# TeemoCaption/FDDM-asr

Hardware: AMD Instinct MI355X
Metric: train-step utterances/sec (10 s @16 kHz, seq_len 256) at 1/2/4/8 MI355X (higher is better)
Workload: dtype bf16; 1 GPU; fddm_zhTW_base C2: WavLM-base + 6L d512 H8 ff2048 decoder, V=8000, T=200, dropout 0.1, n_step_fd=4; global_batch=32, seq_len=256, parallelism=dp1

## Files before the change

fddm-asr_amd/csrc/attention.hip:

```cpp
#include "attn_common.h"

namespace fddm {
namespace attn {


template <typename T> struct Cfg;
template <> struct Cfg<bf16_t> { static constexpr int RB = 128, NSUB = 2, ECH = 8; };
template <> struct Cfg<float> { static constexpr int RB = 256, NSUB = 4, ECH = 4; };

__device__ __forceinline__ int hatt(int k) { return ((k >> 1) & 3) << 2; }

template <typename T>
__device__ __forceinline__ void mma(f32x4_t& c, const uint4& a, const uint4& b);
template <> __device__ __forceinline__ void mma<bf16_t>(f32x4_t& c, const uint4& a, const uint4& b) {
  c = __builtin_amdgcn_mfma_f32_16x16x32_bf16(__builtin_bit_cast(bf16x8_t, a), __builtin_bit_cast(bf16x8_t, b), c, 0, 0, 0);
}
template <> __device__ __forceinline__ void mma<float>(f32x4_t& c, const uint4& a, const uint4& b) {
  c = __builtin_amdgcn_mfma_f32_16x16x4f32(__uint_as_float(a.x), __uint_as_float(b.x), c, 0, 0, 0);
  c = __builtin_amdgcn_mfma_f32_16x16x4f32(__uint_as_float(a.y), __uint_as_float(b.y), c, 0, 0, 0);
  c = __builtin_amdgcn_mfma_f32_16x16x4f32(__uint_as_float(a.z), __uint_as_float(b.z), c, 0, 0, 0);
  c = __builtin_amdgcn_mfma_f32_16x16x4f32(__uint_as_float(a.w), __uint_as_float(b.w), c, 0, 0, 0);
}

template <typename T>
// ... 2197 lines not shown
        uv.y = pk(kok ? dv[d][2] * vsc : 0.f, kok ? dv[d][3] * vsc : 0.f);
        *(uint2*)(dKb + d * 16 + 4 * g) = uk;
        *(uint2*)(dVb + d * 16 + 4 * g) = uv;
      }
    }
  }
  ASTAMP(12);
#ifdef ATTN_STAMPS
  asm volatile("s_waitcnt vmcnt(0)" ::: "memory");
#endif
  ASTAMP(13);
  ARTIME(15);
}

static int g_attn_v6 = 0;
#ifndef A7_FUSED_MAXLQ
#define A7_FUSED_MAXLQ 256
#endif
static bool attn7_enabled() { return g_attn_v6 != 1; }

static int g_last_fwd = AF_NONE, g_last_bwd = AB_NONE;
void attn_note_fwd(int kernel, int dm, int mk, bool kx, bool rel) {
  g_last_fwd = kernel | (dm << 4) | (mk << 6) | ((int)kx << 8) | ((int)rel << 9);
}
void attn_note_bwd(int kernel, int dm, int mk, int np, bool kx) {
  g_last_bwd = kernel | (dm << 4) | (mk << 6) | (np << 9) | ((int)kx << 11);
}
void attn_note_dkv(int kernel, int dm, bool mask, bool kx) {
  const bool same = ((g_last_bwd >> 4) & 3) == dm && (((g_last_bwd >> 11) & 1) != 0) == kx;
  g_last_bwd |= ((same ? kernel : (int)AB_DISAGREE) << 12) | ((int)mask << 8);
// ... 7 lines not shown
      n = v;
    else
      n = 256;
  }
  return n;
}

template <typename T>
static int run(int which, AttnArgs& a, hipStream_t s) {
  constexpr int RB = Cfg<T>::RB;
  const bool drop = a.thr16 != 0, mask = a.key_keep != nullptr || (a.Lk % 64) != 0;
  if constexpr (sizeof(T) == 2) {
    if (which == 0) {
      const bool rel = a.table != nullptr && (a.gate != nullptr || a.graw != nullptr || a.gx != nullptr);
      const int LkP = (a.Lk + 63) / 64 * 64;
      if (rel) {
        if (drop) return (int)hipErrorInvalidValue;
        if (attn7_enabled() && a.Lk <= 1024 && g_attn_v6 != 5) return attn7_fwd(a, s);
        const size_t lds5 = (size_t)2 * 2 * 64 * 128 + (size_t)LkP * 4 + (size_t)(LkP + 128) * 4;
        dim3 grid5((a.Lq + 127) / 128, a.B * a.H);
        if (mask) hipLaunchKernelGGL((fwd5_kernel<true, 2, 2>), grid5, dim3(256), lds5, s, a);
        else hipLaunchKernelGGL((fwd5_kernel<false, 2, 2>), grid5, dim3(256), lds5, s, a);
        attn_note_fwd(AF_FWD5, 0, mask, false, true);
        return (int)hipGetLastError();
      }
      if (a.Lk <= 1024) {
        const int ntiles = LkP / 64, qw = 128;
        const int dm = !drop ? 0 : (a.bits_ready && a.dbits) ? 1 : 2;
        if (attn7_enabled() && (dm != 2 || a.dbits)) {
          if (dm == 2) {
            const int e = attn7_drop_bits(a.dbits, 0, 1, a.B * a.H, a.Lq, a.Lk, a.seed, a.stream, 0, a.thr16,
                                          a.seed_off, s);
            if (e) return e;
// ... 133 lines not shown
FDDM_API int fddm_attn_stamps(unsigned long long* host, long n) {
  return (int)hipMemcpyFromSymbol(host, HIP_SYMBOL(fddm::attn::attn_stamps), n * sizeof(unsigned long long), 0,
                                  hipMemcpyDeviceToHost);
}
FDDM_API int fddm_attn_stamps_clear() {
  static unsigned long long z[8192 * 16];
  return (int)hipMemcpyToSymbol(HIP_SYMBOL(fddm::attn::attn_stamps), z, sizeof(z), 0, hipMemcpyHostToDevice);
}
#endif

FDDM_API int fddm_attn_last_path(void) { return (int)((unsigned)g_last_fwd | ((unsigned)g_last_bwd << 16)); }

FDDM_API int fddm_attn_set_kernels(int v6) {
  const int old = g_attn_v6;
  g_attn_v6 = (v6 >= 1 && v6 <= 5) ? v6 : 0;
  return old;
}

static int attn_fwd_impl(int dtype, const void* Q, long sq, const void* K, long sk, const void* V, long sv, void* O,
                         long so, float* lse, const unsigned char* key_keep, const int* key_len, const float* gate,
                         const float* table, int B, int H, int Lq, int Lk, float scale, float drop_p,
                         unsigned long long seed, unsigned long long stream, unsigned long long* drop_bits,
                         int drop_bits_ready, void* hs) {
  if (table && !gate) return (int)hipErrorInvalidValue;
  attn_note_fwd(AF_NONE, 0, 0, false, false);
  AttnArgs a{};
  a.key_len = key_len;
  a.dbits = (uint64_t*)drop_bits;
  a.bits_ready = drop_bits_ready;
  a.Q = Q; a.K = K; a.V = V; a.Out = O; a.lse = lse;
// ... 130 lines not shown
```

fddm-asr_amd/csrc/attn8.hip:

```cpp
#include "attn7_common.h"

namespace fddm {
namespace attn {

constexpr int A8_NS = 4;
#ifndef A8_RSMFMA
#define A8_RSMFMA 1
#endif
#ifndef A8_WPS
#define A8_WPS 2
#endif

__device__ __forceinline__ void pinv(float& x) { asm volatile("" : "+v"(x)); }
__device__ __forceinline__ void pinv(unsigned& x) { asm volatile("" : "+v"(x)); }
template <int B0, int B1>
__device__ __forceinline__ unsigned keep_pack(float x, float y, unsigned kw) {
  unsigned r, t;
  asm volatile(
      "v_bfe_i32 %1, %3, %5, 1\n\t"
      "v_and_b32 %1, %1, %2\n\t"
      "v_bfe_i32 %0, %3, %6, 1\n\t"
      "v_and_b32 %0, %0, %4\n\t"
      "v_cvt_pk_bf16_f32 %0, %1, %0"
      : "=&v"(r), "=&v"(t)
      : "v"(x), "v"(kw), "v"(y), "i"(B0), "i"(B1));
  return r;
}
#define A8_FENCE() __builtin_amdgcn_sched_barrier(0)

#ifdef A8_STAMPS
#define A8ST(k)                                 \
  do {                                          \
    a8st_[k] = __builtin_amdgcn_s_memtime();  \
  } while (0)
#else
#define A8ST(k) \
  do {          \
  } while (0)
#endif
#if defined(A8_STAMPS) && defined(A8_FINE)
#define A8FS(k)                                                  \
  do {                                                           \
    if (a8pc_ == A8_FINE) a8fs_[k] = __builtin_amdgcn_s_memtime(); \
  } while (0)
#else
#define A8FS(k) \
  do {          \
  } while (0)
#endif

__host__ __device__ __forceinline__ int attn8_fwd_fb_off(int Lk) {
  const int LkP = (Lk + 63) / 64 * 64;
  return (2 * A8_NS * A7_TB + A8_NS * 512 * 4 + 16 + LkP * 4 + 15) / 16 * 16;
}

template <int DM, int MK>
__global__ void __launch_bounds__(256, A8_WPS) fwd8_kernel(AttnArgs a) {
  constexpr bool DROP = DM != 0;
  constexpr int NP = DROP ? 6 : 4;
  extern __shared__ __attribute__((aligned(16))) unsigned char sm8[];
  const int ntiles = (a.Lk + 63) >> 6, LkP = ntiles * 64;
  unsigned char* kst = sm8;
  unsigned char* vst = sm8 + A8_NS * A7_TB;
  unsigned* kbl = (unsigned*)(sm8 + 2 * A8_NS * A7_TB);
  unsigned* mpk = kbl + A8_NS * 512 + 4;
  const int tid = threadIdx.x, lane = tid & 63, w = __builtin_amdgcn_readfirstlane(tid >> 6);
  const int hh = lane >> 5, qi = lane & 31;
  int bxi, bh;
  xcd_tile(bxi, bh);
#ifdef A8_STAMPS
  unsigned long long a8st_[16] = {};
#endif
#if defined(A8_STAMPS) && defined(A8_FINE)
  unsigned long long a8fs_[16] = {};
  int a8pc_ = 0;
#endif
  A8ST(0);
  const int b = bh / a.H, h = bh - b * a.H;
  const int qw0 = bxi * 256 + 64 * w;
  const bf16_t* Qb = (const bf16_t*)a.Q + (long)b * a.Lq * a.sq + h * DH;
  const bf16_t* Kb = (const bf16_t*)a.K + (long)b * a.Lk * a.sk + h * DH;
  const bf16_t* Vb = (const bf16_t*)a.V + (long)b * a.Lk * a.sv + h * DH;
  const unsigned sk2 = (unsigned)a.sk * 2u, sv2 = (unsigned)a.sv * 2u;
  const int nqg = (a.Lq + 31) >> 5, qg0 = 8 * bxi + 2 * w;
  const unsigned* lbits = (const unsigned*)(a.dbits + (long)a.B * a.H * nqg * ntiles * 32);

  unsigned kb8[4] = {1u, 1u, 1u, 1u};
  if constexpr (MK == 2) {
#pragma unroll
    for (int j = 0; j < 4; ++j) {
      const int k = min(4 * tid + j, a.Lk - 1);
      asm volatile("global_load_ubyte %0, %1, off" : "=v"(kb8[j]) : "v"(a.key_keep + (long)b * a.Lk + k) : "memory");
    }
  }
  const int qA = qw0 + qi, qB = qw0 + 32 + qi;
  unsigned char* qst = sm8 + attn8_fwd_fb_off(a.Lk) + w * 16384;
#pragma unroll
  for (int u = 0; u < 8; ++u) {
    const int r = 8 * u + (lane >> 3), pch = lane & 7;
    const unsigned qr = (unsigned)min(qw0 + r, a.Lq - 1);
    dma16_sv(Qb, qr * (unsigned)a.sq * 2u + (unsigned)((pch ^ (r & 7)) << 4), qst + 8 * u * 128);
  }
  const unsigned tmask = ntiles >= 32 ? 0xFFFFFFFFu : ((1u << ntiles) - 1u);
  const int nact = ntiles;
  A8ST(15);

  const unsigned kst_a = lds_addr(kst), vst_a = lds_addr(vst), kbl_a = lds_addr(kbl);
  auto piece = [&](int tt, int st, int k) {
    if (k < 4) {
      const int u = k >> 1, R = 16 * w + 8 * u;
      const int r0 = R + (lane >> 3), pch = lane & 7;
// ... 5 lines not shown
    } else {
      const int c = k - 4;
      dma4_so(lbits, (unsigned)(lb_dword(bh, nqg, ntiles, min(qg0 + c, nqg - 1), tt) + lane) * 4u,
              kbl_a + (st * 512 + (2 * w + c) * 64) * 4);
    }
  };
  unsigned fmask = tmask;
  int flast = 0;
  auto next_fill_tile = [&]() {
    if (fmask) {
      flast = __builtin_ctz(fmask);
      fmask &= fmask - 1u;
    }
    return flast;
  };
  {
    const int t0 = next_fill_tile(), t1 = next_fill_tile();
#pragma unroll
    for (int k = 0; k < NP; ++k) piece(t0, 0, k);
#pragma unroll
    for (int k = 0; k < NP; ++k) piece(t1, 1, k);
  }
  A8ST(11);
  asm volatile("s_waitcnt vmcnt(%4)" : "+v"(kb8[0]), "+v"(kb8[1]), "+v"(kb8[2]), "+v"(kb8[3]) : "n"(NP) : "memory");
  if constexpr (MK != 0) {
    if (4 * tid < LkP) {
      unsigned mv[4];
#pragma unroll
      for (int j = 0; j < 4; ++j) {
        const bool ok = 4 * tid + j < a.Lk && (MK == 1 || (kb8[j] & 0xFFu) != 0);
        mv[j] = pk_bf16(1.f, ok ? 0.f : -INFINITY);
      }
      *(uint4*)(mpk + 4 * tid) = make_uint4(mv[0], mv[1], mv[2], mv[3]);
    }
  }
  __builtin_amdgcn_s_barrier();
  A8ST(1);
  const float sl2 = a.scale * 1.4426950408889634f;
  uint4 qa[4], qb[4];
  {
    const unsigned zA = qA < a.Lq ? 0xFFFFFFFFu : 0u, zB = qB < a.Lq ? 0xFFFFFFFFu : 0u;
    const int rA = qi, rB = qi + 32;
#pragma unroll
    for (int ks = 0; ks < 4; ++ks) {
      const uint4 x = *(const uint4*)(qst + rA * 128 + (((2 * ks + hh) ^ (rA & 7)) << 4));
      const uint4 y = *(const uint4*)(qst + rB * 128 + (((2 * ks + hh) ^ (rB & 7)) << 4));
      qa[ks] = scale_frag(make_uint4(x.x & zA, x.y & zA, x.z & zA, x.w & zA), sl2);
      qb[ks] = scale_frag(make_uint4(y.x & zB, y.y & zB, y.z & zB, y.w & zB), sl2);
    }
  }

  int koff[4];
#pragma unroll
  for (int ks = 0; ks < 4; ++ks) koff[ks] = qi * 128 + (((2 * ks + hh) ^ ((qi >> 1) & 7)) << 4);
  const int vi = lane & 15, vrow = 4 * hh + (vi >> 2);
  int voff[2];
#pragma unroll
  for (int db = 0; db < 2; ++db)
    voff[db] = vrow * 128 + (((8 * db + 4 * ((lane >> 4) & 1) + (vi & 3)) ^ ((vrow & 2) << 2)) << 3);

  float rfA = 0.f, rfB = 0.f;
  f32x16_t oA0 = {}, oA1 = {}, oB0 = {}, oB1 = {};
  constexpr bool RSM = A8_RSMFMA != 0;
  float lsA = 0.f, lsB = 0.f;
  f32x16_t lsum = {};
  uint4 ucar = make_uint4(0, 0, 0, 0);
  const unsigned one2 = 0x3F803F80u, selA1 = qi < 16 ? one2 : 0u, selB1 = qi < 16 ? 0u : one2;
  const uint4 selA = make_uint4(selA1, selA1, selA1, selA1), selB = make_uint4(selB1, selB1, selB1, selB1);
  f32x16_t sA, sB;
  uint4 pA[2], pB[2];
  pB[0] = pB[1] = make_uint4(0, 0, 0, 0);
  const uint4 q5init = hh ? make_uint4(0, 0, 0, 0) : make_uint4(pk_bf16(0.f, 1.f), 0u, 0u, 0u);
  uint4 q5A = q5init, q5B = q5init;
  unsigned kwA = 0xFFFFFFFFu, kwB = 0xFFFFFFFFu;
  uint4 kf[4], vf[2][2];
  uint4 k5 = make_uint4(0, 0, 0, 0);
  const unsigned lo32 = hh ? 0u : 0xFFFFFFFFu;
  auto mk5 = [&](int key0) {
    unsigned mk = pk_bf16(1.f, 0.f);
    if constexpr (MK != 0) mk = mpk[key0 + qi];
    return make_uint4(mk & lo32, 0u, 0u, 0u);
  };
  unsigned mkr = 0;
  auto mk5_read = [&](int key0) {
    if constexpr (MK != 0) mkr = mpk[key0 + qi];
  };
  auto mk5_set = [&]() {
    unsigned mk = pk_bf16(1.f, 0.f);
    if constexpr (MK != 0) mk = mkr;
    k5 = make_uint4(mk & lo32, 0u, 0u, 0u);
// ... 28 lines not shown
    if constexpr (DROP) v = keep_pack<lb_bit(kb, 2 * i), lb_bit(kb, 2 * i + 1)>(x, y, kw);
    else v = pk_bf16(x, y);
    pset(p, ic, v);
  };
  auto first_ref = [&](const f32x16_t& s, float& rf, uint4& q5) {
    float tm = fmaxf(s[0], s[1]);
#pragma unroll
    for (int r = 2; r < 16; r += 2) tm = fmaxf(tm, fmaxf(s[r], s[r + 1]));
    tm = xmax32(tm);
    rf = (tm == -INFINITY) ? 0.f : __uint_as_float(((unsigned)pk_bf16(tm, 0.f)) << 16);
    q5 = hh ? make_uint4(0, 0, 0, 0) : make_uint4(pk_bf16(-rf, 1.f), 0u, 0u, 0u);
  };

  auto phase = [&](f32x16_t& SX, const uint4 (&qX)[4], const uint4& q5X, f32x16_t& oY0, f32x16_t& oY1,
                   const uint4 (&pY)[2], const f32x16_t& sZ, float dZ, uint4 (&pZ)[2], float& lZ,
                   const uint4& selZ, const uint4& selP, unsigned kwZ, auto kbc, auto&& rd, auto&& dm) {
    constexpr int KB = decltype(kbc)::value;
    float ex[8], ey[8], la, lb;
    unsigned sh[8], u[8], mk[8];
    auto expo = [&](auto ic) {
      constexpr int i = decltype(ic)::value;
#ifndef A8_NOEXP
      ex[i] = __builtin_amdgcn_exp2f(sZ[2 * i] - dZ);
      ey[i] = __builtin_amdgcn_exp2f(sZ[2 * i + 1] - dZ);
#else
      ex[i] = sZ[2 * i] - dZ;
      ey[i] = sZ[2 * i + 1] - dZ;
#endif
      pinv(ex[i]);
      pinv(ey[i]);
      if constexpr (DROP) {
        sh[i] = kwZ << (8 * KB + i);
        pinv(sh[i]);
      }
    };
    auto fin = [&](auto ic) {
      constexpr int i = decltype(ic)::value;
      if constexpr (!RSM) {
        if constexpr (i == 0) {
          la = ex[0];
          lb = ey[0];
        } else {
// ... 14 lines not shown
        pinv(mk[i]);
      } else {
        pset(pZ, ic, u[i]);
      }
    };
    auto apply = [&](auto ic) {
      constexpr int i = decltype(ic)::value;
      if constexpr (DROP) {
        unsigned v = u[i] & mk[i];
        pinv(v);
        pset(pZ, ic, v);
      }
    };
    auto stages = [&](auto cc) {
      constexpr int c = decltype(cc)::value;
      if constexpr (c < 8) expo(std::integral_constant<int, c>{});
      if constexpr (c >= 1) fin(std::integral_constant<int, c - 1>{});
      if constexpr (c >= 2) apply(std::integral_constant<int, c - 2>{});
      if constexpr (c == 8) {
        apply(std::integral_constant<int, 7>{});
        if constexpr (!RSM) lZ += la + lb;
      }
    };
    auto rsum = [&](auto cc) {
      constexpr int c = decltype(cc)::value;
      if constexpr (RSM && c == 1) lsum = mfma32(selP, ucar, lsum);
      if constexpr (RSM && c == 6) lsum = mfma32(selZ, make_uint4(u[0], u[1], u[2], u[3]), lsum);
    };
#if defined(A8_STAMPS) && defined(A8_FINE)
    ++a8pc_;
// ... 16 lines not shown
      A8FS(ks + 2);
    });
    SX = acc;
    static_for<0, 4>([&](auto pc) {
      constexpr int pi = decltype(pc)::value;
      if constexpr ((pi & 1) == 0) oY0 = mfma32(vf[pi >> 1][0], pY[pi >> 1], oY0);
      else oY1 = mfma32(vf[pi >> 1][1], pY[pi >> 1], oY1);
      rsum(std::integral_constant<int, 5 + pi>{});
      stages(std::integral_constant<int, 5 + pi>{});
      rd(std::integral_constant<int, 5 + pi>{});
      dm(std::integral_constant<int, 5 + pi>{});
      A8_FENCE();
      A8FS(pi + 6);
    });
    if constexpr (RSM) ucar = make_uint4(u[4], u[5], u[6], u[7]);
  };

  unsigned cmask = tmask;
  int t = __builtin_ctz(cmask);
  cmask &= cmask - 1u;
  int st = 0;
  if (nact > 0) {
  {
#pragma unroll
    for (int ks = 0; ks < 4; ++ks) kf[ks] = *(const uint4*)(kst + koff[ks]);
    k5 = mk5(64 * t);
    if constexpr (DROP) {
      kwA = kbl[(2 * w) * 64 + lane];
      kwB = kbl[(2 * w + 1) * 64 + lane];
    }
    f32x16_t acc = mfma32(k5, q5A, f32x16_t{});
#pragma unroll
    for (int ks = 0; ks < 4; ++ks) acc = mfma32(kf[ks], qa[ks], acc);
    sA = acc;
#pragma unroll
    for (int c = 0; c < 4; ++c) rdv(vst, c);
  }
  int fidx = 2, ftile = next_fill_tile();
  auto dm_first = [&](auto base, auto cc) {
    constexpr int c = decltype(cc)::value, k = decltype(base)::value + c / 3;
    if constexpr (c % 3 == 1 && k < NP) piece(ftile, fidx & 3, k);
  };
  auto dm_none = [&](auto) {};
  first_ref(sA, rfA, q5A);
  phase(sB, qb, q5B, oB0, oB1, pB, sA, rfA, pA, lsA, selA, selB, kwA, std::integral_constant<int, 0>{},
        [&](auto cc) {
          constexpr int c = decltype(cc)::value;
          if constexpr (c == 1) mk5_read(64 * t + 32);
          if constexpr (c == 8) mk5_set();
          if constexpr (c >= 5) kf[c - 5] = *(const uint4*)(kst + koff[c - 5] + 32 * 128);
        },
        [&](auto cc) { dm_first(std::integral_constant<int, 0>{}, cc); });
  first_ref(sB, rfB, q5B);
  phase(sA, qa, q5A, oA0, oA1, pA, sB, rfB, pB, lsB, selB, selA, kwB, std::integral_constant<int, 0>{},
        [&](auto cc) {
          constexpr int c = decltype(cc)::value;
          if constexpr (c < 4) rdv(vst, c);
        },
        [&](auto cc) { dm_first(std::integral_constant<int, 3>{}, cc); });
  A8ST(2);
  auto dm_span = [&](auto base, auto cc) {
    constexpr int c = decltype(cc)::value, k = decltype(base)::value + (c == 6 ? 1 : 0);
    if constexpr ((c == 2 || c == 6) && k < NP) piece(ftile, fidx & 3, k);
  };
  for (int i = 0;; ++i) {
    const bool more = cmask != 0u;
    int tn = t, stn = st;
    unsigned kwAn = 0xFFFFFFFFu, kwBn = 0xFFFFFFFFu;
    if (more) {
      tn = __builtin_ctz(cmask);
      cmask &= cmask - 1u;
      stn = st == A8_NS - 1 ? 0 : st + 1;
#ifndef A8_NOWAIT
      asm volatile("s_waitcnt vmcnt(%0) lgkmcnt(0)" ::"n"(NP) : "memory");
// ... 16 lines not shown
        kwBn = kbl[stn * 512 + (2 * w + 1) * 64 + lane];
      }
    }
    ++fidx;
    ftile = next_fill_tile();
    {
      const unsigned char* kimn = kst + stn * A7_TB;
      const unsigned char* vimg = vst + st * A7_TB;
      phase(sB, qb, q5B, oB0, oB1, pB, sA, 0.f, pA, lsA, selA, selB, kwA, std::integral_constant<int, 1>{},
            [&](auto cc) {
              constexpr int c = decltype(cc)::value;
              if constexpr (c == 1) mk5_read(64 * tn);
              if constexpr (c == 8) mk5_set();
              if constexpr (c >= 5) kf[c - 5] = *(const uint4*)(kimn + koff[c - 5]);
            },
            [&](auto cc) { dm_span(std::integral_constant<int, 0>{}, cc); });
      phase(sA, qa, q5A, oA0, oA1, pA, sB, 0.f, pB, lsB, selB, selA, kwB, std::integral_constant<int, 1>{},
            [&](auto cc) {
              constexpr int c = decltype(cc)::value;
              if constexpr (c < 4) rdv(vimg + 32 * 128, c);
            },
            [&](auto cc) { dm_span(std::integral_constant<int, 2>{}, cc); });
    }
    if (!more) break;
    t = tn;
    st = stn;
    kwA = kwAn;
    kwB = kwBn;
    {
      const unsigned char* kimg = kst + st * A7_TB;
      const unsigned char* vimg = vst + st * A7_TB;
      phase(sB, qb, q5B, oB0, oB1, pB, sA, 0.f, pA, lsA, selA, selB, kwA, std::integral_constant<int, 0>{},
            [&](auto cc) {
              constexpr int c = decltype(cc)::value;
              if constexpr (c == 1) mk5_read(64 * t + 32);
              if constexpr (c == 8) mk5_set();
              if constexpr (c >= 5) kf[c - 5] = *(const uint4*)(kimg + koff[c - 5] + 32 * 128);
            },
            [&](auto cc) { dm_span(std::integral_constant<int, 4>{}, cc); });
      phase(sA, qa, q5A, oA0, oA1, pA, sB, 0.f, pB, lsB, selB, selA, kwB, std::integral_constant<int, 0>{},
            [&](auto cc) {
              constexpr int c = decltype(cc)::value;
              if constexpr (c < 4) rdv(vimg, c);
            },
            dm_none);
    }
  }
#pragma unroll
  for (int s = 0; s < 2; ++s) {
    oB0 = mfma32(vf[s][0], pB[s], oB0);
    oB1 = mfma32(vf[s][1], pB[s], oB1);
  }
  if constexpr (RSM) lsum = mfma32(selB, ucar, lsum);
  }

  A8ST(12);
  asm volatile("s_waitcnt vmcnt(0)" ::: "memory");
  A8ST(13);
  float ltA = RSM ? lsum[0] : xsum32(lsA), ltB = RSM ? lsum[8] : xsum32(lsB);
#ifdef A8_NOFALLBACK
  if (false) {
#else
  if (nact > 0 && __any(!(ltA <= 0x1p64f && ltA >= 0x1p-40f) || !(ltB <= 0x1p64f && ltB >= 0x1p-40f))) {
#endif
    unsigned char* kp = sm8 + attn8_fwd_fb_off(a.Lk) + w * 16384;
    unsigned char* vp = kp + 8192;
    auto redo = [&](int c, const uint4 (&qX)[4], f32x16_t& o0, f32x16_t& o1, float& l, float& rf) {
      const int qg = min(qg0 + c, nqg - 1);
      float m = -INFINITY;
      rf = 0.f;
      l = 0.f;
      o0 = f32x16_t{};
      o1 = f32x16_t{};
      uint4 q5 = q5init;
      unsigned tm_ = tmask;
      while (tm_) {
        const int tt = __builtin_ctz(tm_);
        tm_ &= tm_ - 1u;
        const int r = 64 * tt + lane, rr = min(r, a.Lk - 1);
#pragma unroll
        for (int ch = 0; ch < 8; ++ch) {
          const uint4 kx = *(const uint4*)(Kb + (long)rr * a.sk + 8 * ch);
          const uint4 vx = *(const uint4*)(Vb + (long)rr * a.sv + 8 * ch);
          *(uint4*)(kp + lane * 128 + ((ch ^ ((lane >> 1) & 7)) << 4)) = kx;
          *(uint4*)(vp + lane * 128 + ((ch ^ vsw(lane)) << 4)) = vx;
        }
        unsigned kw = 0xFFFFFFFFu;
        if constexpr (DROP) kw = lbits[lb_dword(bh, nqg, ntiles, qg, tt) + lane];
        static_for<0, 2>([&](auto kbc) {
          constexpr int kb = decltype(kbc)::value;
          const uint4 k5_ = mk5(64 * tt + 32 * kb);
          f32x16_t sc = mfma32(k5_, q5, f32x16_t{});
#pragma unroll
          for (int ks = 0; ks < 4; ++ks) sc = mfma32(*(const uint4*)(kp + koff[ks] + kb * 32 * 128), qX[ks], sc);
          float tmx = fmaxf(sc[0], sc[1]);
#pragma unroll
          for (int rr2 = 2; rr2 < 16; rr2 += 2) tmx = fmaxf(tmx, fmaxf(sc[rr2], sc[rr2 + 1]));
          tmx = xmax32(tmx) + rf;
          const float mn = fmaxf(m, tmx);
          float rn = rf;
          if (mn != -INFINITY) rn = __uint_as_float(((unsigned)pk_bf16(mn, 0.f)) << 16);
          const float alpha = (m == -INFINITY) ? 0.f : __builtin_amdgcn_exp2f(rf - rn);
          l *= alpha;
          o0 *= alpha;
          o1 *= alpha;
          uint4 pp[2];
          float la = 0.f, lb = 0.f;
          static_for<0, 8>([&](auto ic) { sm_pair_f32(sc, rn - rf, kw, pp, la, lb, kbc, ic); });
          l += la + lb;
          m = mn;
          rf = rn;
          q5 = hh ? make_uint4(0, 0, 0, 0) : make_uint4(pk_bf16(-rf, 1.f), 0u, 0u, 0u);
#pragma unroll
          for (int s = 0; s < 2; ++s) {
            const int rb = (32 * kb + 16 * s) * 128;
            o0 = mfma32(join_tr(tr_read(vp + voff[0] + rb), tr_read(vp + voff[0] + rb + 1024)), pp[s], o0);
            o1 = mfma32(join_tr(tr_read(vp + voff[1] + rb), tr_read(vp + voff[1] + rb + 1024)), pp[s], o1);
          }
        });
      }
      l = xsum32(l);
    };
    redo(0, qa, oA0, oA1, ltA, rfA);
    redo(1, qb, oB0, oB1, ltB, rfB);
  }
  bf16_t* Ob = (bf16_t*)a.Out + (long)b * a.Lq * a.so + h * DH;
#pragma unroll
  for (int c = 0; c < 2; ++c) {
    const float lt = c ? ltB : ltA;
    const float rf = c ? rfB : rfA;
    const float inv = (lt > 0.f) ? (DROP ? a.drop_scale : 1.f) / lt : NAN;
    const int q = qw0 + 32 * c + qi;
    bf16_t* orow = Ob + (long)min(q, a.Lq - 1) * a.so;
#pragma unroll
    for (int db = 0; db < 2; ++db) {
      const f32x16_t& oo = c ? (db ? oB1 : oB0) : (db ? oA1 : oA0);
#pragma unroll
      for (int gp = 0; gp < 2; ++gp) {
        unsigned p0[2], p1[2];
#pragma unroll
        for (int j = 0; j < 2; ++j) {
          p0[j] = pk_bf16(oo[8 * gp + 2 * j] * inv, oo[8 * gp + 2 * j + 1] * inv);
          p1[j] = pk_bf16(oo[8 * gp + 4 + 2 * j] * inv, oo[8 * gp + 4 + 2 * j + 1] * inv);
        }
        const auto s0 = __builtin_amdgcn_permlane32_swap(p0[0], p1[0], false, false);
        const auto s1 = __builtin_amdgcn_permlane32_swap(p0[1], p1[1], false, false);
        const uint4 v = make_uint4(s0[0], s1[0], s0[1], s1[1]);
// ... 10 lines not shown
    unsigned long long* dst = (unsigned long long*)(Ob + (long)(bxi * 256) * a.so);
#pragma unroll
    for (int k = 0; k < 16; ++k) dst[k] = a8st_[k];
#ifdef A8_FINE
    unsigned long long* dst2 = (unsigned long long*)(Ob + (long)(bxi * 256 + 1) * a.so);
#pragma unroll
    for (int k = 0; k < 16; ++k) dst2[k] = a8fs_[k];
#endif
  }
#endif
}

#ifndef A8_LDS_FLOOR
#define A8_LDS_FLOOR 0
#endif
size_t attn8_fwd_lds(int Lk) {
  const size_t n = (size_t)attn8_fwd_fb_off(Lk) + 4 * 16384;
  return n > (size_t)A8_LDS_FLOOR ? n : (size_t)A8_LDS_FLOOR;
}

int attn8_fwd(AttnArgs& a, hipStream_t s) {
  if (a.Lk > 1024 || a.Lk <= 0 || a.Lq <= 0) return (int)hipErrorInvalidValue;
  const int dm = a.thr16 == 0 ? 0 : 1;
  const int mk = a.key_keep != nullptr ? 2 : (a.Lk % 64) != 0 ? 1 : 0;
  const size_t lds = attn8_fwd_lds(a.Lk);
  dim3 grid((a.Lq + 255) / 256, a.B * a.H);
#define FWD8(D, M) hipLaunchKernelGGL((fwd8_kernel<D, M>), grid, dim3(256), lds, s, a)
  if (dm) { if (mk == 2) FWD8(1, 2); else if (mk == 1) FWD8(1, 1); else FWD8(1, 0); }
  else { if (mk == 2) FWD8(0, 2); else if (mk == 1) FWD8(0, 1); else FWD8(0, 0); }
#undef FWD8
  attn_note_fwd(AF_FWD8, dm, mk, false, false);
  return (int)hipGetLastError();
}

}
}
```

fddm-asr_amd/csrc/attn_common.h:

```cpp
#pragma once
#include "common.h"

FDDM_API long fddm_attn_drop_words(int B, int H, int Lq, int Lk);

namespace fddm {
namespace attn {

__device__ __forceinline__ void xcd_tile(int& bx, int& by) {
  const int nx = gridDim.x, n = nx * gridDim.y;
  const int L = blockIdx.x + blockIdx.y * nx;
  const int x = L & 7, j = L >> 3, q = n >> 3, r = n & 7;
  const int W = (x < r ? x * (q + 1) : r * (q + 1) + (x - r) * q) + j;
  by = W / nx;
  bx = W - by * nx;
}


constexpr int DH = 64;

__device__ __forceinline__ int kc_off(int RB, int r, int c) { return r * RB + ((c ^ ((r >> 1) & 7)) << 4); }

__device__ __forceinline__ float xmax16(float x) {
  const auto r = __builtin_amdgcn_permlane16_swap(__float_as_uint(x), __float_as_uint(x), false, false);
  return fmaxf(__uint_as_float(r[0]), __uint_as_float(r[1]));
// ... 59 lines not shown
  asm volatile("s_mov_b32 m0, %1\n\tglobal_load_lds_dwordx4 %0, off" ::"v"(src), "s"(la) : "memory", "m0");
}
__device__ __forceinline__ void pin16(uint4& x) {
  u32x4v_t v = __builtin_bit_cast(u32x4v_t, x);
  asm volatile("" : "+v"(v));
  x = __builtin_bit_cast(uint4, v);
}

enum { AF_NONE = 0, AF_FWD7, AF_FWD8, AF_FWD6, AF_FWD2, AF_FWD5, AF_GENERIC };
enum { AB_NONE = 0, AB_BWDF7, AB_V7, AB_V2, AB_BWD3S, AB_V4, AB_GENERIC, AB_DISAGREE = 15 };
void attn_note_fwd(int kernel, int dm, int mk, bool kx, bool rel);
void attn_note_bwd(int kernel, int dm, int mk, int np, bool kx);
void attn_note_dkv(int kernel, int dm, bool mask, bool kx);

int attn7_fwd(AttnArgs& a, hipStream_t s);
int attn8_fwd(AttnArgs& a, hipStream_t s);
int attn7_dq(AttnArgs& a, hipStream_t s);
int attn7_dkv(AttnArgs& a, hipStream_t s);
int attn7_bwdf(AttnArgs& a, hipStream_t s);
int attn7_drop_bits(uint64_t* out, long site_words, int nsites, int BH, int Lq, int Lk, uint64_t seed,
                    uint64_t stream0, uint64_t stream_step, unsigned thr16, const uint64_t* seed_off, hipStream_t s);
long attn7_drop_words(int B, int H, int Lq, int Lk);

}
}
```

fddm-asr_amd/fddm_hip/_lib.py:

```python
from __future__ import annotations

import ctypes
import os
import re

_HERE = os.path.dirname(os.path.abspath(__file__))
LIB_PATH = os.environ.get("FDDM_HIP_LIB", os.path.join(_HERE, "libfddm_hip.so"))
_HEADER_CANDIDATES = [
    os.path.join(os.path.dirname(os.path.dirname(_HERE)), "include", "fddm_hip.h"),
    os.path.join(os.path.dirname(_HERE), "include", "fddm_hip.h"),
]


def header_path() -> str:
    for p in _HEADER_CANDIDATES:
        if os.path.exists(p):
            return p
    raise FileNotFoundError("include/fddm_hip.h not found next to the package")


def _ctype(t: str):
    t = t.strip()
    if "*" in t:
        return ctypes.c_void_p
# ... 39 lines not shown
    global _lib, _decls
    if _lib is None:
        if not os.path.exists(LIB_PATH):
            raise ImportError(f"libfddm_hip.so not built ({LIB_PATH}); run `make -C fddm-asr_amd` or "
                              "__graft_entry__.build(). There is no CPU fallback.")
        L = ctypes.CDLL(LIB_PATH)
        _decls = parse_header()
        for name, (res, args) in _decls.items():
            f = getattr(L, name)
            f.restype = res
            f.argtypes = args
        _lib = L
        ak = os.environ.get("FDDM_ATTN_KERNELS")
        if ak:
            L.fddm_attn_set_kernels({"auto": 0, "v6": 1, "nofused": 2, "fwd7": 3, "fwd8": 4, "relfwd5": 5}[ak])
    return _lib


def declared_symbols():
    return sorted(parse_header().keys())


def call(name: str, *args):
    f = getattr(lib(), name)
    rc = f(*args)
    if rc != 0:
        msg = lib().fddm_error_string(rc)
        raise RuntimeError(f"{name} failed: hipError {rc} ({msg.decode() if msg else '?'})")
    return rc
```

include/fddm_hip.h:

```cpp
#ifndef FDDM_HIP_H
#define FDDM_HIP_H
#ifdef __cplusplus
extern "C" {
#endif

int fddm_abi_version(void);
const char* fddm_error_string(int code);

int fddm_gemm(int dtype, int a_dtype, int a_kc, int b_kc, int epi, int out_dtype, const void* A, long lda, long Mi,
              long sAb, const void* B, long ldb, void* C, long ldc, void* C2, const float* bias, float alpha, long M,
              long N, long K, unsigned long long seed, unsigned long long stream, float drop_p, float* colsum,
              void* hip_stream);

int fddm_linear_dx_rope(const void* dy, long ldy, const void* w, long ldw, float* dx, long lddx, const float* cs,
                        const float* sn, long M, long N, long K, long L, void* hip_stream);

int fddm_gemm_persistent_cap(int cap);

int fddm_gemm_dw_grouped(int n, const void* const* dy, const long* ldy, const void* const* x, const long* ldx,
                         float* const* dw, const long* lddw, float* const* db, const long* M, const long* N,
                         const long* K, long kchunk, void* hip_stream);

int fddm_conv1d_gemm(int dtype, int epi, const void* x, long lda, long sAb, long Tin, long Cg, long cstride,
                     long cpad, const void* W, void* out, long ldc, const float* bias, long Bn, long Tout, long N,
// ... 97 lines not shown
                     void* hip_stream);
int fddm_lfd_std_bwd(int zt_dtype, const float* dzt, const void* zt, const float* inv_std, float* dz, long B, long C,
                     void* hip_stream);
int fddm_lfd_loss(const float* Cm, float* loss, long D, float lam, void* hip_stream);
int fddm_lfd_dloss(int out_dtype, const float* Cm, const float* gscale, void* dC, long D, float lam, void* hip_stream);
int fddm_lfd_colstat(const float* z, float* out, const float* mean_sum, float inv_n, long B, long C, void* hip_stream);
int fddm_lfd_std_apply(int out_dtype, const float* z, void* zt, float* inv_std, const float* s1, const float* s2,
                       float inv_n, float eps, long B, long C, void* hip_stream);
int fddm_lfd_bwd_colstat(int zt_dtype, const float* dzt, const void* zt, float* out, long B, long C, void* hip_stream);
int fddm_lfd_std_bwd_apply(int zt_dtype, const float* dzt, const void* zt, const float* inv_std, const float* sums,
                           float inv_n, float scale, float* dz, long B, long C, void* hip_stream);

int fddm_gemm_force_path(int path);
int fddm_gemm_last_path(void);
int fddm_attn_set_kernels(int v6);
int fddm_attn_last_path(void);


int fddm_set_seed_offset(const unsigned long long* off);

int fddm_grad_sumsq(const long* chunk_tensor, const long* chunk_start, const long* numel, const float* const* g,
                    long nchunks, float* total, void* hip_stream);
int fddm_adamw(const long* chunk_tensor, const long* chunk_start, const long* numel, float* const* p,
               const float* const* g, float* const* m, float* const* v, unsigned short* const* pbf,
               float* const* step, long ntensors, long nchunks, const float* total, float max_norm, float lr,
               float lr_wd, float b1, float b2, float eps, int* skipped, int zero_g, float grad_scale,
               void* hip_stream);

int fddm_rows_mean(int dtype, const void* x, float* out, long B, long S, long d, void* hip_stream);
int fddm_time_embed(const long* t, float* emb, long B, long d, float max_steps, void* hip_stream);
// ... 22 lines not shown
```

Before: 3425 utterances/s.

## Add relative-position-bias variant of fwd8 attention kernel for WavLM gated bias

```diff
diff --git a/fddm-asr_amd/csrc/attention.hip b/fddm-asr_amd/csrc/attention.hip
--- a/fddm-asr_amd/csrc/attention.hip
+++ b/fddm-asr_amd/csrc/attention.hip
@@ -2235,6 +2235,7 @@
 }
 
 static int g_attn_v6 = 0;
+static int g_wavlm_fwd = 0;
 #ifndef A7_FUSED_MAXLQ
 #define A7_FUSED_MAXLQ 256
 #endif
@@ -2272,9 +2273,18 @@
     if (which == 0) {
       const bool rel = a.table != nullptr && (a.gate != nullptr || a.graw != nullptr || a.gx != nullptr);
       const int LkP = (a.Lk + 63) / 64 * 64;
+      if (a.table != nullptr && !rel) return (int)hipErrorInvalidValue;
       if (rel) {
         if (drop) return (int)hipErrorInvalidValue;
-        if (attn7_enabled() && a.Lk <= 1024 && g_attn_v6 != 5) return attn7_fwd(a, s);
+        if (attn7_enabled() && a.Lk <= 1024 && g_attn_v6 != 5) {
+          const bool can8 = !a.key_keep && !a.key_len && a.gx && !a.gate && !a.graw && a.Lk <= A8_REL_MAXLK &&
+                            a.Lq <= a.Lk;
+          const long nh = (long)a.B * a.H, ncu = attn_cu_count();
+          const long load8 = (nh * ((a.Lq + 255) / 256) + ncu - 1) / ncu * 256;
+          const long load7 = (nh * ((a.Lq + 127) / 128) + ncu - 1) / ncu * 128;
+          const bool use8 = can8 && g_attn_v6 != 3 && g_wavlm_fwd == 0 && (g_attn_v6 == 4 || load8 <= load7);
+          return use8 ? attn8_fwd(a, s) : attn7_fwd(a, s);
+        }
         const size_t lds5 = (size_t)2 * 2 * 64 * 128 + (size_t)LkP * 4 + (size_t)(LkP + 128) * 4;
         dim3 grid5((a.Lq + 127) / 128, a.B * a.H);
         if (mask) hipLaunchKernelGGL((fwd5_kernel<true, 2, 2>), grid5, dim3(256), lds5, s, a);
@@ -2438,6 +2448,12 @@
 FDDM_API int fddm_attn_set_kernels(int v6) {
   const int old = g_attn_v6;
   g_attn_v6 = (v6 >= 1 && v6 <= 5) ? v6 : 0;
+  return old;
+}
+
+FDDM_API int fddm_attn_set_wavlm_fwd(int fwd7_only) {
+  const int old = g_wavlm_fwd;
+  g_wavlm_fwd = fwd7_only == 1 ? 1 : 0;
   return old;
 }
 
diff --git a/fddm-asr_amd/csrc/attn8.hip b/fddm-asr_amd/csrc/attn8.hip
--- a/fddm-asr_amd/csrc/attn8.hip
+++ b/fddm-asr_amd/csrc/attn8.hip
@@ -28,6 +28,24 @@
 }
 #define A8_FENCE() __builtin_amdgcn_sched_barrier(0)
 
+__device__ __forceinline__ u32x4v_t gload16(const void* p) {
+  u32x4v_t v;
+  asm volatile("global_load_dwordx4 %0, %1, off" : "=v"(v) : "v"(p) : "memory");
+  return v;
+}
+__device__ __forceinline__ unsigned gload4(const void* p) {
+  unsigned v;
+  asm volatile("global_load_dword %0, %1, off" : "=v"(v) : "v"(p) : "memory");
+  return v;
+}
+__device__ __forceinline__ void pin4v(u32x4v_t& x) { asm volatile("" : "+v"(x)); }
+typedef unsigned a8_u32x2 __attribute__((ext_vector_type(2)));
+__device__ __forceinline__ a8_u32x2 lds_ld64(unsigned a) {
+  typedef __attribute__((address_space(3))) const volatile a8_u32x2* lp_t;
+  return *(lp_t)(size_t)a;
+}
+constexpr int A8_BPAD = 288;
+
 #ifdef A8_STAMPS
 #define A8ST(k)                                 \
   do {                                          \
@@ -54,8 +72,9 @@
   return (2 * A8_NS * A7_TB + A8_NS * 512 * 4 + 16 + LkP * 4 + 15) / 16 * 16;
 }
 
-template <int DM, int MK>
+template <int DM, int MK, bool REL = false>
 __global__ void __launch_bounds__(256, A8_WPS) fwd8_kernel(AttnArgs a) {
+  static_assert(!REL || (DM == 0 && MK != 2), "the bias build has no dropout and no key-padding bytes");
   constexpr bool DROP = DM != 0;
   constexpr int NP = DROP ? 6 : 4;
   extern __shared__ __attribute__((aligned(16))) unsigned char sm8[];
@@ -63,7 +82,7 @@
   unsigned char* kst = sm8;
   unsigned char* vst = sm8 + A8_NS * A7_TB;
   unsigned* kbl = (unsigned*)(sm8 + 2 * A8_NS * A7_TB);
-  unsigned* mpk = kbl + A8_NS * 512 + 4;
+  unsigned* mpk = kbl + (REL ? 0 : A8_NS * 512) + 4;
   const int tid = threadIdx.x, lane = tid & 63, w = __builtin_amdgcn_readfirstlane(tid >> 6);
   const int hh = lane >> 5, qi = lane & 31;
   int bxi, bh;
@@ -94,7 +113,7 @@
     }
   }
   const int qA = qw0 + qi, qB = qw0 + 32 + qi;
-  unsigned char* qst = sm8 + attn8_fwd_fb_off(a.Lk) + w * 16384;
+  unsigned char* qst = REL ? (w < 2 ? kst : vst) + (2 + (w & 1)) * A7_TB : sm8 + attn8_fwd_fb_off(a.Lk) + w * 16384;
 #pragma unroll
   for (int u = 0; u < 8; ++u) {
     const int r = 8 * u + (lane >> 3), pch = lane & 7;
@@ -130,10 +149,35 @@
     }
     return flast;
   };
+  constexpr int CLP = REL ? A8_BPAD : 0;
+  const int CL = LkP + CLP;
+  float* bcp = (float*)(mpk + LkP);
+  u32x4v_t gxr[2][4], gwr[2][8];
+  auto rel_loads = [&]() {
+    if constexpr (REL) {
+#pragma unroll
+      for (int c = 0; c < 2; ++c) {
+        const long qc = min(qw0 + 32 * c + qi, a.Lq - 1);
+        const bf16_t* xr = (const bf16_t*)a.gx + ((long)b * a.Lq + qc) * a.sgx + h * DH + 32 * hh;
+#pragma unroll
+        for (int u = 0; u < 4; ++u) gxr[c][u] = gload16(xr + 8 * u);
+#pragma unroll
+        for (int u = 0; u < 8; ++u) gwr[c][u] = gload16(a.gw + 64 * c + 32 * hh + 4 * u);
+      }
+      const float* tabh = a.table + (long)h * (2 * a.Lk - 1);
+      const unsigned bcp_a = lds_addr(bcp);
+      for (int g = w; g < 2 * CL / 64; g += 4) {
+        const int i = 64 * g + lane, c = i >= CL ? 1 : 0;
+        const int ti = (a.Lk - 1) - (bxi * 256 + 255) + (i - c * CL) + c;
+        dma4_so(tabh, (unsigned)min(max(ti, 0), 2 * a.Lk - 2) * 4u, bcp_a + 256u * (unsigned)g);
+      }
+    }
+  };
   {
     const int t0 = next_fill_tile(), t1 = next_fill_tile();
 #pragma unroll
     for (int k = 0; k < NP; ++k) piece(t0, 0, k);
+    rel_loads();
 #pragma unroll
     for (int k = 0; k < NP; ++k) piece(t1, 1, k);
   }
@@ -150,8 +194,48 @@
       *(uint4*)(mpk + 4 * tid) = make_uint4(mv[0], mv[1], mv[2], mv[3]);
     }
   }
+  float g2A = 0.f, g2B = 0.f;
+  unsigned blA = 0, blB = 0;
+  auto bias_off = [&](int c) {
+    const int jq = 255 - (64 * w + 32 * c + qi);
+    return (jq & 1) * CL + (jq & ~1) + 4 * hh;
+  };
   __builtin_amdgcn_s_barrier();
   A8ST(1);
+  if constexpr (REL) {
+#pragma unroll
+    for (int c = 0; c < 2; ++c) {
+#pragma unroll
+      for (int u = 0; u < 4; ++u) pin4v(gxr[c][u]);
+#pragma unroll
+      for (int u = 0; u < 8; ++u) pin4v(gwr[c][u]);
+    }
+    const float ba = a.gw[128], bb = a.gw[129], gc = a.gconst[h];
+    auto gate2 = [&](const u32x4v_t (&xv)[4], bool qv) {
+      float sa = 0.f, sb = 0.f;
+#pragma unroll
+      for (int c = 0; c < 4; ++c) {
+#pragma unroll
+        for (int j = 0; j < 2; ++j) {
+          const u32x4v_t A = gwr[0][2 * c + j], Bw = gwr[1][2 * c + j];
+          const float e0 = __uint_as_float(xv[c][2 * j] << 16), e1 = __uint_as_float(xv[c][2 * j] & 0xFFFF0000u);
+          const float e2 = __uint_as_float(xv[c][2 * j + 1] << 16), e3 = __uint_as_float(xv[c][2 * j + 1] & 0xFFFF0000u);
+          sa = fmaf(e0, __uint_as_float(A[0]), fmaf(e1, __uint_as_float(A[1]), fmaf(e2, __uint_as_float(A[2]),
+                                                                                    fmaf(e3, __uint_as_float(A[3]), sa))));
+          sb = fmaf(e0, __uint_as_float(Bw[0]), fmaf(e1, __uint_as_float(Bw[1]), fmaf(e2, __uint_as_float(Bw[2]),
+                                                                                      fmaf(e3, __uint_as_float(Bw[3]), sb))));
+        }
+      }
+      sa = xsum32(sa) + ba;
+      sb = xsum32(sb) + bb;
+      const float ga = 1.f / (1.f + __expf(-sa)), gb = 1.f / (1.f + __expf(-sb));
+      return (qv ? ga * (gb * gc - 1.f) + 2.f : 0.f) * 1.4426950408889634f;
+    };
+    g2A = gate2(gxr[0], qA < a.Lq);
+    g2B = gate2(gxr[1], qB < a.Lq);
+    blA = lds_addr(bcp) + 4u * (unsigned)bias_off(0);
+    blB = lds_addr(bcp) + 4u * (unsigned)bias_off(1);
+  }
   const float sl2 = a.scale * 1.4426950408889634f;
   uint4 qa[4], qb[4];
   {
@@ -164,6 +248,15 @@
       qa[ks] = scale_frag(make_uint4(x.x & zA, x.y & zA, x.z & zA, x.w & zA), sl2);
       qb[ks] = scale_frag(make_uint4(y.x & zB, y.y & zB, y.z & zB, y.w & zB), sl2);
     }
+  }
+  if constexpr (REL) {
+#pragma unroll
+    for (int ks = 0; ks < 4; ++ks) {
+      pin16(qa[ks]);
+      pin16(qb[ks]);
+    }
+    asm volatile("s_waitcnt lgkmcnt(0)" ::: "memory");
+    __builtin_amdgcn_s_barrier();
   }
 
   int koff[4];
@@ -190,6 +283,7 @@
   uint4 q5A = q5init, q5B = q5init;
   unsigned kwA = 0xFFFFFFFFu, kwB = 0xFFFFFFFFu;
   uint4 kf[4], vf[2][2];
+  a8_u32x2 bw[8];
   uint4 k5 = make_uint4(0, 0, 0, 0);
   const unsigned lo32 = hh ? 0u : 0xFFFFFFFFu;
   auto mk5 = [&](int key0) {
@@ -248,18 +342,30 @@
 
   auto phase = [&](f32x16_t& SX, const uint4 (&qX)[4], const uint4& q5X, f32x16_t& oY0, f32x16_t& oY1,
                    const uint4 (&pY)[2], const f32x16_t& sZ, float dZ, uint4 (&pZ)[2], float& lZ,
-                   const uint4& selZ, const uint4& selP, unsigned kwZ, auto kbc, auto&& rd, auto&& dm) {
+                   const uint4& selZ, const uint4& selP, unsigned kwZ, auto kbc, auto&& rd, auto&& dm, float gZ,
+                   unsigned& blZ, unsigned blN, auto bmc) {
     constexpr int KB = decltype(kbc)::value;
+    constexpr int BM = REL ? decltype(bmc)::value : 0;
     float ex[8], ey[8], la, lb;
     unsigned sh[8], u[8], mk[8];
+    auto bread = [&](auto cc) {
+      constexpr int c = decltype(cc)::value;
+      if constexpr ((BM & 1) && c <= 5) bw[c + 2] = lds_ld64(blZ + 32 * ((c + 2) >> 1) + 8 * ((c + 2) & 1));
+      if constexpr ((BM & 2) && c >= 7) bw[c - 7] = lds_ld64(blN + 8 * (c - 7));
+    };
     auto expo = [&](auto ic) {
       constexpr int i = decltype(ic)::value;
+      float s0 = sZ[2 * i], s1 = sZ[2 * i + 1];
+      if constexpr ((BM & 1) != 0) {
+        s0 = fmaf(gZ, __uint_as_float(bw[i][0]), s0);
+        s1 = fmaf(gZ, __uint_as_float(bw[i][1]), s1);
+      }
 #ifndef A8_NOEXP
-      ex[i] = __builtin_amdgcn_exp2f(sZ[2 * i] - dZ);
-      ey[i] = __builtin_amdgcn_exp2f(sZ[2 * i + 1] - dZ);
+      ex[i] = __builtin_amdgcn_exp2f(s0 - dZ);
+      ey[i] = __builtin_amdgcn_exp2f(s1 - dZ);
 #else
-      ex[i] = sZ[2 * i] - dZ;
-      ey[i] = sZ[2 * i + 1] - dZ;
+      ex[i] = s0 - dZ;
+      ey[i] = s1 - dZ;
 #endif
       pinv(ex[i]);
       pinv(ey[i]);
@@ -304,6 +410,7 @@
     };
     auto stages = [&](auto cc) {
       constexpr int c = decltype(cc)::value;
+      bread(cc);
       if constexpr (c < 8) expo(std::integral_constant<int, c>{});
       if constexpr (c >= 1) fin(std::integral_constant<int, c - 1>{});
       if constexpr (c >= 2) apply(std::integral_constant<int, c - 2>{});
@@ -350,7 +457,23 @@
       A8FS(pi + 6);
     });
     if constexpr (RSM) ucar = make_uint4(u[4], u[5], u[6], u[7]);
-  };
+    if constexpr (REL) blZ += 128u;
+  };
+  auto bias_first = [&](f32x16_t& s, float g, unsigned bl) {
+    a8_u32x2 t[8];
+    static_for<0, 8>([&](auto ic) {
+      constexpr int i = decltype(ic)::value;
+      t[i] = lds_ld64(bl + 32 * (i >> 1) + 8 * (i & 1));
+    });
+    static_for<0, 8>([&](auto ic) {
+      constexpr int i = decltype(ic)::value;
+      s[2 * i] = fmaf(g, __uint_as_float(t[i][0]), s[2 * i]);
+      s[2 * i + 1] = fmaf(g, __uint_as_float(t[i][1]), s[2 * i + 1]);
+    });
+  };
+  constexpr std::integral_constant<int, 0> BM0{};
+  constexpr std::integral_constant<int, 2> BM2{};
+  constexpr std::integral_constant<int, 3> BM3{};
 
   unsigned cmask = tmask;
   int t = __builtin_ctz(cmask);
@@ -378,6 +501,7 @@
     if constexpr (c % 3 == 1 && k < NP) piece(ftile, fidx & 3, k);
   };
   auto dm_none = [&](auto) {};
+  if constexpr (REL) bias_first(sA, g2A, blA);
   first_ref(sA, rfA, q5A);
   phase(sB, qb, q5B, oB0, oB1, pB, sA, rfA, pA, lsA, selA, selB, kwA, std::integral_constant<int, 0>{},
         [&](auto cc) {
@@ -386,14 +510,15 @@
           if constexpr (c == 8) mk5_set();
           if constexpr (c >= 5) kf[c - 5] = *(const uint4*)(kst + koff[c - 5] + 32 * 128);
         },
-        [&](auto cc) { dm_first(std::integral_constant<int, 0>{}, cc); });
+        [&](auto cc) { dm_first(std::integral_constant<int, 0>{}, cc); }, 0.f, blA, 0u, BM0);
+  if constexpr (REL) bias_first(sB, g2B, blB);
   first_ref(sB, rfB, q5B);
   phase(sA, qa, q5A, oA0, oA1, pA, sB, rfB, pB, lsB, selB, selA, kwB, std::integral_constant<int, 0>{},
         [&](auto cc) {
           constexpr int c = decltype(cc)::value;
           if constexpr (c < 4) rdv(vst, c);
         },
-        [&](auto cc) { dm_first(std::integral_constant<int, 3>{}, cc); });
+        [&](auto cc) { dm_first(std::integral_constant<int, 3>{}, cc); }, 0.f, blB, blA, BM2);
   A8ST(2);
   auto dm_span = [&](auto base, auto cc) {
     constexpr int c = decltype(cc)::value, k = decltype(base)::value + (c == 6 ? 1 : 0);
@@ -440,13 +565,13 @@
               if constexpr (c == 8) mk5_set();
               if constexpr (c >= 5) kf[c - 5] = *(const uint4*)(kimn + koff[c - 5]);
             },
-            [&](auto cc) { dm_span(std::integral_constant<int, 0>{}, cc); });
+            [&](auto cc) { dm_span(std::integral_constant<int, 0>{}, cc); }, g2A, blA, blB, BM3);
       phase(sA, qa, q5A, oA0, oA1, pA, sB, 0.f, pB, lsB, selB, selA, kwB, std::integral_constant<int, 1>{},
             [&](auto cc) {
               constexpr int c = decltype(cc)::value;
               if constexpr (c < 4) rdv(vimg + 32 * 128, c);
             },
-            [&](auto cc) { dm_span(std::integral_constant<int, 2>{}, cc); });
+            [&](auto cc) { dm_span(std::integral_constant<int, 2>{}, cc); }, g2B, blB, blA, BM3);
     }
     if (!more) break;
     t = tn;
@@ -463,13 +588,13 @@
               if constexpr (c == 8) mk5_set();
               if constexpr (c >= 5) kf[c - 5] = *(const uint4*)(kimg + koff[c - 5] + 32 * 128);
             },
-            [&](auto cc) { dm_span(std::integral_constant<int, 4>{}, cc); });
+            [&](auto cc) { dm_span(std::integral_constant<int, 4>{}, cc); }, g2A, blA, blB, BM3);
       phase(sA, qa, q5A, oA0, oA1, pA, sB, 0.f, pB, lsB, selB, selA, kwB, std::integral_constant<int, 0>{},
             [&](auto cc) {
               constexpr int c = decltype(cc)::value;
               if constexpr (c < 4) rdv(vimg, c);
             },
-            dm_none);
+            dm_none, g2B, blB, blA, BM3);
     }
   }
 #pragma unroll
@@ -483,15 +608,20 @@
   A8ST(12);
   asm volatile("s_waitcnt vmcnt(0)" ::: "memory");
   A8ST(13);
+  if constexpr (REL) {
+    asm volatile("s_waitcnt lgkmcnt(0)" ::: "memory");
+    __builtin_amdgcn_s_barrier();
+  }
   float ltA = RSM ? lsum[0] : xsum32(lsA), ltB = RSM ? lsum[8] : xsum32(lsB);
 #ifdef A8_NOFALLBACK
   if (false) {
 #else
   if (nact > 0 && __any(!(ltA <= 0x1p64f && ltA >= 0x1p-40f) || !(ltB <= 0x1p64f && ltB >= 0x1p-40f))) {
 #endif
-    unsigned char* kp = sm8 + attn8_fwd_fb_off(a.Lk) + w * 16384;
-    unsigned char* vp = kp + 8192;
-    auto redo = [&](int c, const uint4 (&qX)[4], f32x16_t& o0, f32x16_t& o1, float& l, float& rf) {
+    unsigned char* kp = REL ? kst + w * A7_TB : sm8 + attn8_fwd_fb_off(a.Lk) + w * 16384;
+    unsigned char* vp = REL ? vst + w * A7_TB : kp + 8192;
+    auto redo = [&](int c, const uint4 (&qX)[4], f32x16_t& o0, f32x16_t& o1, float& l, float& rf, float g2,
+                    int boff) {
       const int qg = min(qg0 + c, nqg - 1);
       float m = -INFINITY;
       rf = 0.f;
@@ -519,6 +649,11 @@
           f32x16_t sc = mfma32(k5_, q5, f32x16_t{});
 #pragma unroll
           for (int ks = 0; ks < 4; ++ks) sc = mfma32(*(const uint4*)(kp + koff[ks] + kb * 32 * 128), qX[ks], sc);
+          if constexpr (REL) {
+            const float* bp = bcp + boff + 64 * tt + 32 * kb;
+#pragma unroll
+            for (int r2 = 0; r2 < 16; ++r2) sc[r2] = fmaf(g2, bp[8 * (r2 >> 2) + (r2 & 3)], sc[r2]);
+          }
           float tmx = fmaxf(sc[0], sc[1]);
 #pragma unroll
           for (int rr2 = 2; rr2 < 16; rr2 += 2) tmx = fmaxf(tmx, fmaxf(sc[rr2], sc[rr2 + 1]));
@@ -547,8 +682,8 @@
       }
       l = xsum32(l);
     };
-    redo(0, qa, oA0, oA1, ltA, rfA);
-    redo(1, qb, oB0, oB1, ltB, rfB);
+    redo(0, qa, oA0, oA1, ltA, rfA, g2A, bias_off(0));
+    redo(1, qb, oB0, oB1, ltB, rfB, g2B, bias_off(1));
   }
   bf16_t* Ob = (bf16_t*)a.Out + (long)b * a.Lq * a.so + h * DH;
 #pragma unroll
@@ -556,7 +691,9 @@
     const float lt = c ? ltB : ltA;
     const float rf = c ? rfB : rfA;
     const float inv = (lt > 0.f) ? (DROP ? a.drop_scale : 1.f) / lt : NAN;
-    const int q = qw0 + 32 * c + qi;
+    int qie = qi;
+    if constexpr (REL) asm volatile("" : "+v"(qie));
+    const int q = qw0 + 32 * c + qie;
     bf16_t* orow = Ob + (long)min(q, a.Lq - 1) * a.so;
 #pragma unroll
     for (int db = 0; db < 2; ++db) {
@@ -597,7 +734,9 @@
 #ifndef A8_LDS_FLOOR
 #define A8_LDS_FLOOR 0
 #endif
-size_t attn8_fwd_lds(int Lk) {
+size_t attn8_fwd_lds(int Lk, bool rel = false) {
+  const int LkP = (Lk + 63) / 64 * 64;
+  if (rel) return (size_t)2 * A8_NS * A7_TB + 16 + (size_t)LkP * 4 + (size_t)2 * (LkP + A8_BPAD) * 4;
   const size_t n = (size_t)attn8_fwd_fb_off(Lk) + 4 * 16384;
   return n > (size_t)A8_LDS_FLOOR ? n : (size_t)A8_LDS_FLOOR;
 }
@@ -606,8 +745,18 @@
   if (a.Lk > 1024 || a.Lk <= 0 || a.Lq <= 0) return (int)hipErrorInvalidValue;
   const int dm = a.thr16 == 0 ? 0 : 1;
   const int mk = a.key_keep != nullptr ? 2 : (a.Lk % 64) != 0 ? 1 : 0;
-  const size_t lds = attn8_fwd_lds(a.Lk);
+  const bool rel = a.table != nullptr && (a.gate != nullptr || a.graw != nullptr || a.gx != nullptr);
+  if (rel && (dm || mk == 2 || a.key_len || a.gate || a.graw || !a.gx || !a.gw || !a.gconst ||
+              a.Lk > A8_REL_MAXLK || a.Lq > a.Lk))
+    return (int)hipErrorInvalidValue;
+  const size_t lds = attn8_fwd_lds(a.Lk, rel);
   dim3 grid((a.Lq + 255) / 256, a.B * a.H);
+  if (rel) {
+    if (mk == 1) hipLaunchKernelGGL((fwd8_kernel<0, 1, true>), grid, dim3(256), lds, s, a);
+    else hipLaunchKernelGGL((fwd8_kernel<0, 0, true>), grid, dim3(256), lds, s, a);
+    attn_note_fwd(AF_FWD8, 0, mk, false, true);
+    return (int)hipGetLastError();
+  }
 #define FWD8(D, M) hipLaunchKernelGGL((fwd8_kernel<D, M>), grid, dim3(256), lds, s, a)
   if (dm) { if (mk == 2) FWD8(1, 2); else if (mk == 1) FWD8(1, 1); else FWD8(1, 0); }
   else { if (mk == 2) FWD8(0, 2); else if (mk == 1) FWD8(0, 1); else FWD8(0, 0); }
diff --git a/fddm-asr_amd/csrc/attn_common.h b/fddm-asr_amd/csrc/attn_common.h
--- a/fddm-asr_amd/csrc/attn_common.h
+++ b/fddm-asr_amd/csrc/attn_common.h
@@ -97,6 +97,7 @@
 void attn_note_dkv(int kernel, int dm, bool mask, bool kx);
 
 int attn7_fwd(AttnArgs& a, hipStream_t s);
+constexpr int A8_REL_MAXLK = 512;
 int attn8_fwd(AttnArgs& a, hipStream_t s);
 int attn7_dq(AttnArgs& a, hipStream_t s);
 int attn7_dkv(AttnArgs& a, hipStream_t s);
diff --git a/fddm-asr_amd/fddm_hip/_lib.py b/fddm-asr_amd/fddm_hip/_lib.py
--- a/fddm-asr_amd/fddm_hip/_lib.py
+++ b/fddm-asr_amd/fddm_hip/_lib.py
@@ -77,6 +77,9 @@
         ak = os.environ.get("FDDM_ATTN_KERNELS")
         if ak:
             L.fddm_attn_set_kernels({"auto": 0, "v6": 1, "nofused": 2, "fwd7": 3, "fwd8": 4, "relfwd5": 5}[ak])
+        wa = os.environ.get("FDDM_WAVLM_ATTN")
+        if wa:
+            L.fddm_attn_set_wavlm_fwd({"auto": 0, "fwd7": 1}[wa])
     return _lib
 
 
diff --git a/include/fddm_hip.h b/include/fddm_hip.h
--- a/include/fddm_hip.h
+++ b/include/fddm_hip.h
@@ -135,6 +135,7 @@
 int fddm_gemm_force_path(int path);
 int fddm_gemm_last_path(void);
 int fddm_attn_set_kernels(int v6);
+int fddm_attn_set_wavlm_fwd(int fwd7_only);
 int fddm_attn_last_path(void);
 
 
```

Result: no change. 3448 utterances/s, median of 6 (+0.7%).
